# PKU-EPIC/GraspNeRF

Hardware: AMD Instinct MI355X
Metric: scenes/sec TSDF+render fwd, 6-view 40^3 grid (higher is better)
Workload: dtype f32

## Files before the change

### graspnerf_amd/_lib.py

```python
import ctypes as C
import os

_HERE = os.path.dirname(os.path.abspath(__file__))
LIB_PATH = os.path.join(_HERE, 'csrc', os.environ.get('GNR_LIB', 'libgnr.so'))

GNR_OK, GNR_ERR_ARG, GNR_ERR_SHAPE, GNR_ERR_HIP, GNR_ERR_WORKSPACE = 0, -1, -2, -3, -4
ERRORS = {-1: 'GNR_ERR_ARG', -2: 'GNR_ERR_SHAPE', -3: 'GNR_ERR_HIP', -4: 'GNR_ERR_WORKSPACE'}

c_float_p = C.POINTER(C.c_float)


class GnrScene(C.Structure):
    _fields_ = [('B', C.c_int), ('V', C.c_int), ('H', C.c_int), ('W', C.c_int), ('fh', C.c_int), ('fw', C.c_int),
                ('imgs', C.c_void_p), ('img_feats', C.c_void_p), ('ray_feats', C.c_void_p),
                ('poses', C.c_void_p), ('Ks', C.c_void_p), ('depth_range', C.c_void_p), ('use_vis', C.c_int), ('options', C.c_uint)]


OPTIONS = {'fp32_chain': 0x001, 'feature_grad_fixed': 0x002, 'view1_one_wavefront': 0x004, 'view2_one_wavefront': 0x008,
           'ray_order_morton': 0x010, 'poison_partials': 0x020, 'direct_scatter': 0x040, 'geo_dual_fp32': 0x080, 'test_lose_partner': 0x100, 'static_tiles': 0x200, 'split_launch': 0x400,
           'sample_order_natural': 0x800}
GNR_STATUS_LOST_PARTNER = 16


class GnrRays(C.Structure):
# ... 51 lines not shown
        getattr(L, name).argtypes = [C.c_void_p, C.c_void_p, C.c_void_p]
        getattr(L, name).restype = C.c_int
    L.gnr_layout_offset.argtypes = [C.c_char_p]
    L.gnr_layout_offset.restype = C.c_int
    L.gnr_workspace_bytes.argtypes = [C.POINTER(GnrScene), C.c_int, C.c_int, C.c_int]
    L.gnr_workspace_bytes.restype = C.c_size_t
    L.gnr_prepare.argtypes = [C.POINTER(GnrScene), C.c_void_p, C.c_size_t, C.c_void_p]
    L.gnr_prepare.restype = C.c_int
    L.gnr_range_status.argtypes = [C.POINTER(GnrScene), C.c_void_p, C.c_size_t, C.POINTER(C.c_uint), C.c_void_p]
    L.gnr_range_status.restype = C.c_int
    L.gnr_status_words_offset.argtypes = [C.POINTER(GnrScene)]
    L.gnr_status_words_offset.restype = C.c_size_t
    L.gnr_sample_volume_fwd.argtypes = [C.POINTER(GnrScene), C.c_void_p, C.c_int, C.c_void_p, C.c_void_p,
                                        C.c_void_p, C.c_void_p, C.c_size_t, C.c_void_p]
    L.gnr_sample_volume_fwd.restype = C.c_int
    L.gnr_debug_volume_chain.argtypes = [C.POINTER(GnrScene), C.c_void_p, C.c_int, C.c_void_p, C.c_void_p,
                                         C.c_void_p, C.c_size_t, C.c_void_p]
    L.gnr_debug_volume_chain.restype = C.c_int
    L.gnr_depth_mean_fwd.argtypes = [C.POINTER(GnrScene), C.c_void_p, C.c_int, C.c_void_p, C.c_void_p,
                                     C.c_void_p, C.c_size_t, C.c_void_p]
    L.gnr_depth_mean_fwd.restype = C.c_int
    L.gnr_merge_depths.argtypes = [C.c_void_p, C.c_int, C.c_void_p, C.c_int, C.c_void_p, C.c_int, C.c_void_p]
    L.gnr_merge_depths.restype = C.c_int
    L.gnr_render_by_depth_fwd.argtypes = [C.POINTER(GnrScene), C.POINTER(GnrRays), C.c_void_p, C.c_int, C.c_void_p,
                                          C.POINTER(GnrRenderOut), C.c_void_p, C.c_size_t, C.c_void_p]
    L.gnr_render_by_depth_fwd.restype = C.c_int
    L.gnr_debug_render_by_depth_perm.argtypes = [C.POINTER(GnrScene), C.POINTER(GnrRays), C.c_void_p, C.c_int, C.c_void_p,
                                                 C.POINTER(GnrRenderOut), C.c_void_p, C.c_void_p, C.c_size_t, C.c_void_p]
    L.gnr_debug_render_by_depth_perm.restype = C.c_int
    L.gnr_debug_sample_order.argtypes = [C.c_void_p, C.c_int, C.c_int, C.c_void_p, C.c_void_p]
    L.gnr_debug_sample_order.restype = C.c_int
    L.gnr_sample_order_host.argtypes = [C.c_void_p, C.c_int, C.c_void_p]
    L.gnr_sample_order_host.restype = C.c_int
    L.gnr_sample_order_offsets.argtypes = [C.POINTER(GnrScene), C.c_int, C.c_int, C.POINTER(C.c_size_t), C.POINTER(C.c_size_t)]
    L.gnr_sample_order_offsets.restype = C.c_int
    L.gnr_render_rays_fwd.argtypes = [C.POINTER(GnrScene), C.POINTER(GnrRays), C.c_void_p, C.c_void_p,
                                      C.POINTER(GnrRenderOut), C.POINTER(GnrRenderOut), C.c_void_p, C.c_void_p,
                                      C.c_void_p, C.c_size_t, C.c_void_p]
    L.gnr_render_rays_fwd.restype = C.c_int
    L.gnr_head_canonical_floats.restype = C.c_int
    L.gnr_head_packed_floats.restype = C.c_int
    L.gnr_pack_grasp_head.argtypes = [c_float_p, c_float_p]
    L.gnr_pack_grasp_head.restype = C.c_int
    L.gnr_grasp_head_workspace_bytes.argtypes = [C.c_int, C.c_int]
    L.gnr_grasp_head_workspace_bytes.restype = C.c_size_t
    L.gnr_grasp_head_fwd.argtypes = [C.c_int, C.c_int, C.c_void_p, C.c_void_p, C.c_void_p, C.c_void_p, C.c_void_p,
                                     C.c_void_p, C.c_size_t, C.c_void_p]
    L.gnr_grasp_head_fwd.restype = C.c_int
    L.gnr_head_last_error.restype = C.c_char_p
    L.gnr_conv3d_bwd_weight.argtypes = [C.c_void_p] * 3 + [C.c_int] * 7 + [C.c_void_p]
    L.gnr_conv3d_same_bwd_weight.argtypes = [C.c_void_p] * 3 + [C.c_int] * 7 + [C.c_void_p, C.c_size_t, C.c_void_p]
    L.gnr_conv3d_same_bwd_weight_workspace_bytes.argtypes = [C.c_int] * 7
    L.gnr_conv3d_same_bwd_weight_workspace_bytes.restype = C.c_size_t
    L.gnr_conv3d_same_bwd_weight.restype = C.c_int
    L.gnr_conv3d_same_workspace_bytes.argtypes = [C.c_int] * 3
    L.gnr_conv3d_same_workspace_bytes.restype = C.c_size_t
    L.gnr_conv3d_same.argtypes = [C.c_void_p] * 4 + [C.c_int] * 8 + [C.c_void_p, C.c_size_t, C.c_void_p]
    L.gnr_conv3d_same.restype = C.c_int
    L.gnr_conv3d_tap_mask_words.argtypes = [C.c_int] * 2
    L.gnr_conv3d_tap_mask_words.restype = C.c_size_t
    L.gnr_conv3d_tap_mask.argtypes = [C.c_void_p, C.c_void_p, C.c_int, C.c_int, C.c_int, C.c_void_p]
    L.gnr_conv3d_tap_mask.restype = C.c_int
    L.gnr_conv3d_same_masked.argtypes = [C.c_void_p] * 4 + [C.c_int] * 8 + [C.c_void_p, C.c_void_p, C.c_size_t, C.c_void_p]
    L.gnr_conv3d_same_masked.restype = C.c_int
    L.gnr_conv3d_same_bwd_weight_masked.argtypes = [C.c_void_p] * 3 + [C.c_int] * 7 + [C.c_void_p, C.c_void_p, C.c_size_t, C.c_void_p]
    L.gnr_conv3d_same_bwd_weight_masked.restype = C.c_int
# ... 61 lines not shown
    L.gnr_timing_begin_only.argtypes = [C.c_char_p]
    L.gnr_timing_begin_only.restype = C.c_int
    L.gnr_timing_end.argtypes = [C.c_char_p, C.c_size_t]
    L.gnr_timing_end.restype = C.c_int
    L.gnr_chain_timing_end.argtypes = [c_float_p, C.POINTER(C.c_int)]
    L.gnr_chain_timing_end.restype = C.c_int
    L.gnr_img_last_error.restype = C.c_char_p
    L.gnr_instnorm_act.argtypes = [C.c_void_p] * 7 + [C.c_longlong, C.c_int, C.c_int, C.c_float, C.c_int, C.c_void_p]
    L.gnr_instnorm_act.restype = C.c_int
    L.gnr_instnorm_act_bwd.argtypes = [C.c_void_p] * 12 + [C.c_longlong, C.c_int, C.c_int, C.c_int, C.c_void_p]
    L.gnr_instnorm_act_bwd.restype = C.c_int
    for fn in (L.gnr_reflect_pad2d, L.gnr_reflect_pad2d_bwd):
        fn.argtypes = [C.c_void_p, C.c_void_p, C.c_longlong, C.c_int, C.c_int, C.c_int, C.c_void_p]
        fn.restype = C.c_int
    L.gnr_upsample2x_bilinear.argtypes = [C.c_void_p, C.c_void_p, C.c_longlong, C.c_int, C.c_int, C.c_void_p]
    L.gnr_upsample2x_bilinear.restype = C.c_int
    L.gnr_ingest_tables_bytes.argtypes = [C.c_int, C.c_int]
    L.gnr_ingest_tables_bytes.restype = C.c_size_t
    L.gnr_ingest_tables_host.argtypes = [C.c_int] * 4 + [C.c_void_p]
    L.gnr_ingest_tables_host.restype = C.c_int
    L.gnr_ingest_u8.argtypes = [C.c_void_p] + [C.c_int] * 4 + [C.c_size_t, C.c_size_t, C.c_void_p, C.c_void_p, C.c_int, C.c_int, C.c_void_p]
    L.gnr_ingest_u8.restype = C.c_int
    L.gnr_ingest_last_error.restype = C.c_char_p
    L.gnr_last_error.restype = C.c_char_p
    L.gnr_dominant_kernel_name.restype = C.c_char_p
    L.gnr_debug_fill_lds.argtypes = [C.c_uint, C.c_void_p]
    L.gnr_debug_fill_lds.restype = C.c_int
    _lib = L
    return L


EXPORTED = ['gnr_canonical_weights_floats', 'gnr_packed_weights_floats', 'gnr_pack_weights', 'gnr_pack_vis_decoder', 'gnr_pack_vis_decoder_bwd', 'gnr_canonical_vis_floats', 'gnr_pack_weights_device', 'gnr_pack_weights_bwd_device', 'gnr_pack_vis_decoder_device', 'gnr_pack_vis_decoder_bwd_device', 'gnr_layout_offset', 'gnr_workspace_bytes',
            'gnr_prepare', 'gnr_range_status', 'gnr_status_words_offset', 'gnr_sample_volume_fwd', 'gnr_debug_volume_chain', 'gnr_depth_mean_fwd', 'gnr_merge_depths', 'gnr_render_by_depth_fwd', 'gnr_render_rays_fwd',
            'gnr_debug_render_by_depth_perm', 'gnr_debug_sample_order', 'gnr_sample_order_host', 'gnr_sample_order_offsets',
            'gnr_dominant_kernel_name', 'gnr_last_error', 'gnr_time_chain_kernel', 'gnr_head_canonical_floats',
            'gnr_head_packed_floats', 'gnr_pack_grasp_head', 'gnr_grasp_head_workspace_bytes', 'gnr_grasp_head_fwd',
            'gnr_head_last_error', 'gnr_chain_timing_begin', 'gnr_chain_timing_end', 'gnr_timing_begin', 'gnr_timing_begin_only', 'gnr_timing_end', 'gnr_grasp_select_workspace_bytes',
            'gnr_grasp_select_fwd', 'gnr_post_last_error', 'gnr_packed_bwd_floats', 'gnr_pack_weights_bwd',
            'gnr_depth_mean_bwd_workspace_bytes', 'gnr_depth_mean_bwd', 'gnr_sample_volume_train_workspace_bytes',
            'gnr_train_workspace_layout', 'gnr_sample_volume_fwd_train', 'gnr_sample_volume_bwd',
            'gnr_render_chain_train_workspace_bytes', 'gnr_render_chain_fwd_train', 'gnr_render_chain_bwd', 'gnr_conv3d_bwd_weight', 'gnr_conv3d_same_workspace_bytes', 'gnr_conv3d_same', 'gnr_conv3d_tap_mask_words', 'gnr_conv3d_tap_mask', 'gnr_conv3d_same_masked', 'gnr_conv3d_same_bwd_weight_masked', 'gnr_conv3d_same_bwd_weight', 'gnr_conv3d_same_bwd_weight_workspace_bytes',
            'gnr_render_tail_fwd_train', 'gnr_ray_tail_grad_floats', 'gnr_ray_tail_dual_bwd', 'gnr_ray_tail_dual_bwd_workspace_bytes', 'gnr_composite_bwd', 'gnr_composite_bwd_workspace_bytes', 'gnr_geo_dual_fwd', 'gnr_geo_dual_fwd_workspace_bytes', 'gnr_geo_dual_bwd', 'gnr_geo_dual_bwd_workspace_bytes', 'gnr_host_randperm_prefix',
            'gnr_debug_fill_lds', 'gnr_img_last_error', 'gnr_instnorm_act', 'gnr_instnorm_act_bwd', 'gnr_reflect_pad2d', 'gnr_reflect_pad2d_bwd', 'gnr_upsample2x_bilinear',
            'gnr_ingest_tables_bytes', 'gnr_ingest_tables_host', 'gnr_ingest_u8', 'gnr_ingest_last_error']


def check(rc, what):
    if rc != GNR_OK:
        msg = lib().gnr_last_error().decode(errors='replace')
        raise GnrError(f'{what} failed: {ERRORS.get(rc, rc)} ({msg})')


def timing_begin(only=None):
    check(lib().gnr_timing_begin_only(only.encode() if only else None), 'gnr_timing_begin')


def timing_end():
    buf = C.create_string_buffer(1 << 16)
    n = lib().gnr_timing_end(buf, len(buf))
    if n < 0:
        check(n, 'gnr_timing_end')
    out = {}
    for line in buf.value.decode().splitlines():
        label, cnt, ms = line.rsplit(' ', 2)
        out[label] = (int(cnt), float(ms))
    return out
```

### graspnerf_amd/csrc/gnr_capi.inc

```
#include <stdio.h>
#include <string.h>
#include <atomic>
#include <mutex>
#include <type_traits>

#include "../../include/gnr.h"

namespace gnr {

static thread_local char g_err[512] = "";
static int fail(int code, const char* what, hipError_t e = hipSuccess) {
    snprintf(g_err, sizeof(g_err), "%s%s%s", what, e != hipSuccess ? ": " : "", e != hipSuccess ? hipGetErrorString(e) : "");
    return code;
}
#define GNR_HIP(call)                                                         \
    do {                                                                      \
        hipError_t e_ = (call);                                               \
        if (e_ != hipSuccess) return fail(GNR_ERR_HIP, #call, e_);            \
    } while (0)

static inline size_t al256(size_t x) { return (x + 255) & ~(size_t)255; }

static bool attr_needed(std::atomic<unsigned long long>& done) {
    int dev = 0;
// ... 453 lines not shown
}

extern "C" int gnr_sample_volume_fwd(const GnrScene* s, const float* bbox_min, int R, const float* wc, float* sdf_out,
                                     unsigned char* vmask_out, void* ws, size_t ws_bytes, void* stream) {
    if (int rc = check_scene(s)) return rc;
    if (!bbox_min || !wc || !sdf_out || !ws) return fail(GNR_ERR_ARG, "gnr_sample_volume_fwd: null pointer");
    if (R < 2 || R > MAX_DN) return fail(GNR_ERR_SHAPE, "volume_res must be in 2..64");
    return volume_impl(s, bbox_min, R, wc, sdf_out, vmask_out, ws, ws_bytes, (hipStream_t)stream, true, true, true);
}

extern "C" int gnr_debug_volume_chain(const GnrScene* s, const float* bbox_min, int R, const float* wc, float* dbg,
                                      void* ws, size_t ws_bytes, void* stream) {
    if (int rc = check_scene(s)) return rc;
    if (!bbox_min || !wc || !dbg || !ws) return fail(GNR_ERR_ARG, "gnr_debug_volume_chain: null pointer");
    return volume_impl(s, bbox_min, R, wc, nullptr, nullptr, ws, ws_bytes, (hipStream_t)stream, true, true, false, dbg);
}

static int order_rays(const GnrScene* s, const GnrRays* q, Workspace& w, hipStream_t st, const int** perm_out) {
    *perm_out = nullptr;
    if (!opt(s, GNR_OPT_RAY_ORDER_MORTON) || q->rn > MAX_SORT_RAYS || q->rn < 2) return GNR_OK;
    int shift = 0;
    while (((s->W > s->H ? s->W : s->H) >> shift) > 1024) ++shift;
    if (int rc = launch<k_ray_order>("k_ray_order@render_pass", st, dim3(s->B), dim3(256), 0, q->coords, w.ray_perm, q->rn, shift)) return rc;
    *perm_out = w.ray_perm;
    return GNR_OK;
}

constexpr int SAMPLE_ORDER_MIN_TILES_PER_SLOT = 8;
static bool sample_order_wanted(const GnrScene* s, const Workspace& w, int P) {
    if (opt(s, GNR_OPT_SAMPLE_ORDER_NATURAL) || !w.sample_perm || !w.sample_keys || P > MAX_SORT_SAMPLES) return false;
    const long ntiles = (long)s->B * ((P + 15) / 16), slots = (long)num_cus() * (GNR_CHAIN_THREADS / 64);
    return ntiles >= SAMPLE_ORDER_MIN_TILES_PER_SLOT * slots;
}
static int launch_sample_order(const unsigned char* keys, int* perm, int B, int P, int nkeys, hipStream_t st) {
    return launch<k_sample_order>("k_sample_order@render_pass", st, dim3(B), dim3(1024), 0, keys, perm, P, nkeys);
}
static RayArgs render_ray_args(const GnrScene* s, const GnrRays* q, const float* depth, int dn, const float* wl, const GnrRenderOut* out,
                               const Workspace& w, const float* desc) {
    RayArgs r;
    memset(&r, 0, sizeof(r));
    r.wpk = wl; r.rec = w.rec; r.desc = desc; r.depth = depth; r.colors = out->colors_nr; r.que_dr = q->que_depth_range;
    r.nrays = s->B * q->rn; r.dn = dn; r.rays_per_scene = q->rn;
    r.sdf = out->sdf_values; r.alpha = out->alpha_values; r.hit = out->hit_prob_nr; r.pix = out->pixel_colors_nr;
    r.rdepth = out->render_depth; r.gerr_part = out->sdf_gradient_error ? w.gerr_part : nullptr; r.grad = out->sdf_gradient;
    r.rmask = out->ray_mask; r.view_num = q->ray_mask_view_num; r.point_num = q->ray_mask_point_num;
    r.range_word = w.range_flag ? w.range_flag + RS_RAY_WATCH : nullptr;
    return r;
}
static int render_ray_epilogue(const GnrScene* s, const GnrRays* q, const GnrRenderOut* out, int dn, const Workspace& w, const char* gerr_label,
                               const char* gt_label, bool want_gt, float* gt_also, hipStream_t st) {
    const int B = s->B, rn = q->rn;
    if (out->sdf_gradient_error) {
        const int chunk = q->ray_batch_num > 0 ? q->ray_batch_num : rn;
        if (int rc = launch<k_gerr_reduce>(gerr_label, st, dim3(B, (rn + chunk - 1) / chunk), dim3(256), 0, w.gerr_part, out->sdf_gradient_error, rn, dn, chunk)) return rc;
    }
    if (out->pixel_colors_gt && q->que_imgs && want_gt)
        if (int rc = launch<k_pixel_gt>(gt_label, st, dim3((B * rn + 255) / 256), dim3(256), 0, q->que_imgs, q->coords, out->pixel_colors_gt, rn, s->H, s->W, B, gt_also)) return rc;
    return GNR_OK;
}
static int render_pass(const GnrScene* s, const GnrRays* q, const float* depth, int dn, const float* wl, GnrRenderOut* out,
                       Workspace& w, hipStream_t st, float* fine_depth, int* fine_inds, int fdn, const float* fine_u = nullptr,
                       const int* perm = nullptr, int range_slot = RS_COARSE, float* gt_also = nullptr, bool skip_gt = false, bool gen_depth = false,
                       const int* sample_perm_in = nullptr) {
    if (!out || !out->colors_nr) return fail(GNR_ERR_ARG, "GnrRenderOut.colors_nr is required");
    const int B = s->B, rn = q->rn;
    const int P = rn * dn;
    const bool ordered = !sample_perm_in && sample_order_wanted(s, w, P);
    if (int rc = launch<k_points_rays>("k_points_rays@render_pass", st, dim3((B * P + 255) / 256), dim3(256), 0, q->coords, q->que_pose, q->que_K,
                                       q->que_depth_range, depth, w.desc, rn, dn, B, perm, gen_depth ? const_cast<float*>(depth) : nullptr,
                                       ordered ? w.sample_keys : nullptr, w.viewp, s->V, s->H, s->W)) return rc;
    if (ordered)
        if (int rc = launch_sample_order(w.sample_keys, w.sample_perm, B, P, 1 << s->V, st)) return rc;
    ChainArgs a{wl, w.feat64, s->imgs, w.viewp, w.desc, w.rec, out->colors_nr, out->view_mask, nullptr,
                B, P, s->H, s->W, s->fh, s->fw, 0};
    wire_chain(a, s, w, range_slot);
    a.ray_perm = perm; a.perm_rn = rn; a.perm_dn = dn;
    a.sample_perm = ordered ? w.sample_perm : sample_perm_in;
    if (int rc = launch_chain<true>(s, a, st)) return rc;
    RayArgs r = render_ray_args(s, q, depth, dn, wl, out, w, w.desc);
    r.fine_depth = fine_depth; r.fine_inds = fine_inds; r.fdn = fdn; r.fine_u = fine_u; r.ray_perm = perm;
    if (int rc = launch_ray<true>(r, st)) return rc;
    if (int rc = render_ray_epilogue(s, q, out, dn, w, "k_gerr_reduce@render_pass", "k_pixel_gt@render_pass", !skip_gt, gt_also, st)) return rc;
    if (out->depth && out->depth != depth)
        GNR_HIP(hipMemcpyAsync(out->depth, depth, (size_t)B * P * sizeof(float), hipMemcpyDeviceToDevice, st));
    return GNR_OK;
}

static int check_rays(const GnrRays* q, bool by_depth = false) {
    if (!q || !q->coords || !q->que_pose || !q->que_K || !q->que_depth_range) return fail(GNR_ERR_ARG, "GnrRays: null pointer");
    if (q->rn < 1) return fail(GNR_ERR_SHAPE, "GnrRays: rn must be positive");
    if (!by_depth && (q->dn < 3 || q->dn > MAX_DN || q->fdn < 1 || q->fdn > MAX_DN)) return fail(GNR_ERR_SHAPE, "GnrRays: dn/fdn must be in 3..64");
    if (q->fine_depth_use_all != 0 && q->fine_depth_use_all != 1) return fail(GNR_ERR_ARG, "GnrRays: fine_depth_use_all must be 0 or 1");
    if (q->ray_batch_num < 0) return fail(GNR_ERR_SHAPE, "GnrRays: ray_batch_num must be >= 0");
    return GNR_OK;
}

extern "C" int gnr_render_by_depth_fwd(const GnrScene* s, const GnrRays* q, const float* depth, int dn, const float* wl,
                                       GnrRenderOut* out, void* ws, size_t ws_bytes, void* stream) {
    if (int rc = check_scene(s)) return rc;
    if (int rc = check_rays(q, true)) return rc;
    if (!depth || !wl || !ws) return fail(GNR_ERR_ARG, "gnr_render_by_depth_fwd: null pointer");
    if (dn < 3 || dn > MAX_DN_FWD) return fail(GNR_ERR_SHAPE, "dn must be in 3..128");
    if (int rc = check_points(s, (size_t)q->rn * dn)) return rc;
    Workspace w = carve(s, (size_t)q->rn * dn, q->rn, ws);
    if (ws_bytes < w.total) return fail(GNR_ERR_WORKSPACE, "workspace too small");
    const int* perm = nullptr;
    if (int rc = order_rays(s, q, w, (hipStream_t)stream, &perm)) return rc;
    return render_pass(s, q, depth, dn, wl, out, w, (hipStream_t)stream, nullptr, nullptr, 0, nullptr, perm);
}

extern "C" int gnr_debug_render_by_depth_perm(const GnrScene* s, const GnrRays* q, const float* depth, int dn, const float* wl,
                                              GnrRenderOut* out, const int* sample_perm, void* ws, size_t ws_bytes, void* stream) {
    if (int rc = check_scene(s)) return rc;
    if (int rc = check_rays(q, true)) return rc;
    if (!depth || !wl || !ws || !sample_perm) return fail(GNR_ERR_ARG, "gnr_debug_render_by_depth_perm: null pointer");
    if (dn < 3 || dn > MAX_DN_FWD) return fail(GNR_ERR_SHAPE, "dn must be in 3..128");
    if (int rc = check_points(s, (size_t)q->rn * dn)) return rc;
    Workspace w = carve(s, (size_t)q->rn * dn, q->rn, ws);
    if (ws_bytes < w.total) return fail(GNR_ERR_WORKSPACE, "workspace too small");
    const int* perm = nullptr;
    if (int rc = order_rays(s, q, w, (hipStream_t)stream, &perm)) return rc;
    return render_pass(s, q, depth, dn, wl, out, w, (hipStream_t)stream, nullptr, nullptr, 0, nullptr, perm, RS_COARSE, nullptr, false, false, sample_perm);
}

extern "C" int gnr_debug_sample_order(const unsigned char* keys, int B, int P, int* perm, void* stream) {
    if (!keys || !perm) return fail(GNR_ERR_ARG, "gnr_debug_sample_order: null pointer");
    if (B < 1 || P < 1 || P > MAX_SORT_SAMPLES) return fail(GNR_ERR_SHAPE, "gnr_debug_sample_order: 1 <= P <= 2^18 samples per scene");
    return launch_sample_order(keys, perm, B, P, 256, (hipStream_t)stream);
}
extern "C" int gnr_sample_order_host(const unsigned char* keys, int P, int* perm_out) {
    if (!keys || !perm_out) return fail(GNR_ERR_ARG, "gnr_sample_order_host: null pointer");
    if (P < 1) return fail(GNR_ERR_SHAPE, "gnr_sample_order_host: P must be positive");
    int start[256], hist[256] = {0};
    for (int i = 0; i < P; ++i) ++hist[keys[i]];
    for (int k = 0; k < 256; ++k) {
        start[k] = 0;
        for (int k2 = 0; k2 < 256; ++k2) if (sorder::key_before(k2, k)) start[k] += hist[k2];
    }
    for (int i = 0; i < P; ++i) perm_out[sorder::slot_of(start[keys[i]]++, P)] = i;
    return GNR_OK;
}
extern "C" int gnr_sample_order_offsets(const GnrScene* s, int rn, int dn_max, size_t* keys_off, size_t* perm_off) {
    if (!s || !keys_off || !perm_off) return fail(GNR_ERR_ARG, "gnr_sample_order_offsets: null pointer");
    if (rn < 1 || dn_max < 1) return fail(GNR_ERR_SHAPE, "gnr_sample_order_offsets: rn, dn_max must be positive");
    char* const base = (char*)4096;
    Workspace w = carve(s, (size_t)rn * dn_max, rn, base);
    if ((size_t)rn * dn_max > (size_t)MAX_SORT_SAMPLES) return fail(GNR_ERR_SHAPE, "gnr_sample_order_offsets: more samples per scene than the sort handles");
    *keys_off = (size_t)((char*)w.sample_keys - base); *perm_off = (size_t)((char*)w.sample_perm - base);
    return GNR_OK;
}

extern "C" int gnr_render_rays_fwd(const GnrScene* s, const GnrRays* q, const float* wc, const float* wf, GnrRenderOut* coarse,
                                   GnrRenderOut* fine, const float* fine_depth_in, int* fine_inds_out, void* ws, size_t ws_bytes,
                                   void* stream) {
    if (int rc = check_scene(s)) return rc;
    if (int rc = check_rays(q)) return rc;
    if (!wc || !coarse || !ws || (fine && !wf)) return fail(GNR_ERR_ARG, "gnr_render_rays_fwd: null pointer");
    if (!fine && (fine_depth_in || fine_inds_out)) return fail(GNR_ERR_ARG, "gnr_render_rays_fwd: fine depths / indices without a fine pass");
    hipStream_t st = (hipStream_t)stream;
    const int fine_dn = !fine ? 0 : (q->fine_depth_use_all ? q->dn + q->fdn : q->fdn);
    const int dmax = q->dn > fine_dn ? q->dn : fine_dn;
    if (int rc = check_points(s, (size_t)q->rn * dmax)) return rc;
    Workspace w = carve(s, (size_t)q->rn * dmax, q->rn, ws);
    if (ws_bytes < w.total) return fail(GNR_ERR_WORKSPACE, "workspace too small");
    const int B = s->B;
    float* depth_c = coarse->depth ? coarse->depth : w.depth_c;
    const int* perm = nullptr;
    if (int rc = order_rays(s, q, w, st, &perm)) return rc;
    if (!fine) return render_pass(s, q, depth_c, q->dn, wc, coarse, w, st, nullptr, nullptr, 0, nullptr, perm, RS_COARSE, nullptr, false, true);
    float* depth_f = (fine->depth && !fine_depth_in && !q->fine_depth_use_all) ? fine->depth : w.depth_f;
    const bool one_gt = coarse->pixel_colors_gt && fine->pixel_colors_gt && q->que_imgs && coarse->pixel_colors_gt != fine->pixel_colors_gt;
    if (int rc = render_pass(s, q, depth_c, q->dn, wc, coarse, w, st, depth_f, fine_inds_out, q->fdn, q->fine_u, perm, RS_COARSE,
// ... 583 lines not shown
```

### graspnerf_amd/csrc/gnr_kernels.hip

```cpp
#include <hip/hip_runtime.h>
#include <stdint.h>
#include <type_traits>

#include "gnr_layout.h"
#include "gnr_sample_order.h"

#ifndef GNR_ABLATE
#define GNR_ABLATE 0
#endif

namespace gnr {

typedef float f4 __attribute__((ext_vector_type(4)));
typedef float f2 __attribute__((ext_vector_type(2)));

#define DEV __device__ __forceinline__

DEV f4 mfma16(float a, float b, f4 c) { return __builtin_amdgcn_mfma_f32_16x16x4f32(a, b, c, 0, 0, 0); }
DEV float elu1(float x) { return fmaxf(x, __builtin_amdgcn_fmed3f(__expf(x), 0.f, 1.f) - 1.f); }
constexpr float kLog2e = 1.4426950408889634f, kLn2 = 0.6931471805599453f;
#if GNR_ABLATE & 8
DEV float elu_s(float xs) { return xs; }
#else
DEV float elu_s(float xs) { return fmaxf(xs, fmaf(__builtin_amdgcn_fmed3f(__builtin_amdgcn_exp2f(xs), 0.f, 1.f), kLog2e, -kLog2e)); }
// ... 555 lines not shown
    };
    assemble(0, 1, o.f);
    assemble(2, 3, o.i);
}
DEV void view_dir(const float* __restrict__ vp, const float (&p)[3], const float (&qd)[3], float (&dd)[4]) {
    float d[3] = {p[0] - vp[12], p[1] - vp[13], p[2] - vp[14]};
    const float inr = -__builtin_amdgcn_rsqf(fmaxf(d[0] * d[0] + d[1] * d[1] + d[2] * d[2], 1e-10f));
    d[0] *= inr; d[1] *= inr; d[2] *= inr;
    dd[0] = d[0] - qd[0]; dd[1] = d[1] - qd[1]; dd[2] = d[2] - qd[2];
    dd[3] = d[0] * qd[0] + d[1] * qd[1] + d[2] * qd[2];
}

constexpr int SW = 20;
#ifndef GNR_TWO_QUEUES
#define GNR_TWO_QUEUES 0
#endif
#ifndef GNR_RDF2_PAIRS
#define GNR_RDF2_PAIRS 0
#endif
constexpr int rows_a(int V) { return GNR_TWO_QUEUES ? (V + 1) / 2 : V; }
constexpr int rows_b(int V) { return GNR_TWO_QUEUES ? V / 2 : 0; }

DEV unsigned view_mask_key(const float* __restrict__ viewp_b, const float (&p)[3], int V, int H, int W) {
    const float qd[3] = {0.f, 0.f, 0.f};
    unsigned k = 0;
    for (int v = 0; v < V; ++v) {
        ViewGeom vg;
        project_view<false>(viewp_b + v * VIEWP_FLOATS, p, qd, H, W, vg);
        k |= (vg.m != 0.f ? 1u : 0u) << v;
    }
    return k;
}
constexpr int MAX_SORT_SAMPLES = 1 << 18;
constexpr int SO_DEPTH = 16;
__global__ __launch_bounds__(1024) void k_sample_order(const unsigned char* __restrict__ keys, int* __restrict__ perm, int P, int nkeys) {
    __shared__ int hist[256];
    __shared__ int wbase[16][256];
    const int tid = threadIdx.x, lane = tid & 63, wave = tid >> 6;
    const unsigned char* kb = keys + (size_t)blockIdx.x * P;
    int* pb = perm + (size_t)blockIdx.x * P;
    for (int i = tid; i < 16 * 256; i += 1024) (&wbase[0][0])[i] = 0;
    __syncthreads();
    const int seg = ((P + 16 * 64 - 1) / (16 * 64)) * 64;
    const int s0 = min(P, wave * seg), s1 = min(P, s0 + seg);
    for (int i0 = s0; i0 < s1; i0 += 64 * SO_DEPTH) {
        int kk[SO_DEPTH];
#pragma unroll
        for (int u = 0; u < SO_DEPTH; ++u) { const int i = i0 + u * 64 + lane; kk[u] = i < s1 ? (int)kb[i] : -1; }
#pragma unroll
        for (int u = 0; u < SO_DEPTH; ++u) if (kk[u] >= 0) atomicAdd(&wbase[wave][kk[u]], 1);
    }
    __syncthreads();
    if (tid < nkeys) {
        int t = 0;
        for (int w = 0; w < 16; ++w) t += wbase[w][tid];
        hist[tid] = t;
    }
    __syncthreads();
    if (tid < nkeys) {
        int run = 0;
        for (int k2 = 0; k2 < nkeys; ++k2) if (sorder::key_before(k2, tid)) run += hist[k2];
        for (int w = 0; w < 16; ++w) { const int c = wbase[w][tid]; wbase[w][tid] = run; run += c; }
    }
    __syncthreads();
    volatile int* base = wbase[wave];
    for (int i0 = s0; i0 < s1; i0 += 64 * SO_DEPTH) {
        int kk[SO_DEPTH];
#pragma unroll
        for (int u = 0; u < SO_DEPTH; ++u) { const int i = i0 + u * 64 + lane; kk[u] = i < s1 ? (int)kb[i] : -1; }
#pragma unroll
        for (int u = 0; u < SO_DEPTH; ++u) {
            if (i0 + u * 64 >= s1) break;
            const int k = kk[u];
            const bool ok = k >= 0;
            unsigned long long same = __ballot(ok);
#pragma unroll
            for (int bit = 0; bit < 8; ++bit) {
                const bool on = (k >> bit) & 1;
                const unsigned long long bb = __ballot(on);
                same &= on ? bb : ~bb;
            }
            const int rank = __popcll(same & ((1ull << lane) - 1ull));
            const int pos = ok ? base[k] + rank : 0;
            __builtin_amdgcn_wave_barrier();
            if (ok && rank == 0) base[k] = pos + __popcll(same);
            __builtin_amdgcn_wave_barrier();
            if (ok) pb[sorder::slot_of(pos, P)] = i0 + u * 64 + lane;
        }
    }
}

#ifndef GNR_DYN_TILES
#define GNR_DYN_TILES 1
#endif
#ifndef GNR_VOLUME_POINTS_INLINE
#define GNR_VOLUME_POINTS_INLINE 1
#endif
#ifndef GNR_TAIL_OLD_ONLY
#define GNR_TAIL_OLD_ONLY 0
#endif
#ifndef GNR_DESC_PREFETCH
#define GNR_DESC_PREFETCH 0
#endif
#ifndef GNR_DYN_CTR_INC
#define GNR_DYN_CTR_INC 0
#endif
#ifndef GNR_DYN_TRAIN
#define GNR_DYN_TRAIN 1
#endif
#ifndef GNR_SKIP_MASKED
#define GNR_SKIP_MASKED 1
#endif
#ifndef GNR_CHAIN_THREADS
#define GNR_CHAIN_THREADS 512
#endif
#define GNR_CHAIN_MIN_BLOCKS (GNR_CHAIN_THREADS >= 1024 ? 1 : GNR_CHAIN_THREADS / 256)
#ifndef GNR_WAVE_CLOCK
#define GNR_WAVE_CLOCK 0
#endif
#if GNR_WAVE_CLOCK
__device__ unsigned long long g_wave_clock[2][4096][8];
__device__ unsigned g_tile_clock[2][1 << 17];
// ... 1388 lines not shown
```

### graspnerf_amd/csrc/gnr_sample_order.h

```cpp
#pragma once

#if defined(__HIPCC__)
#define GNR_SO_HD __host__ __device__
#else
#define GNR_SO_HD
#endif

namespace gnr {
namespace sorder {

constexpr int STRIPES = 8;
constexpr int TILE = 16;

GNR_SO_HD inline int popcount8(int k) { k = (k & 0x55) + ((k >> 1) & 0x55); k = (k & 0x33) + ((k >> 2) & 0x33); return (k & 0x0f) + (k >> 4); }

GNR_SO_HD inline bool key_before(int a, int b) {
    const int pa = popcount8(a), pb = popcount8(b);
    return pa != pb ? pa > pb : a > b;
}

GNR_SO_HD inline int stripe_tiles(int tps, int s) { return (tps - s + STRIPES - 1) / STRIPES; }

GNR_SO_HD inline int slot_of(int pos, int P) {
    const int tps = (P + TILE - 1) / TILE;
    const int rem = P - (tps - 1) * TILE;
    const int gshort = tps <= STRIPES ? tps - 1 : STRIPES * (tps / STRIPES) - 1;
    int gi, wi;
    if (pos < TILE * gshort) { gi = pos / TILE; wi = pos % TILE; }
    else if (pos < TILE * gshort + rem) { gi = gshort; wi = pos - TILE * gshort; }
    else { const int q = pos + TILE - rem; gi = q / TILE; wi = q % TILE; }
    const int s = gi % STRIPES;
    int tile = gi / STRIPES;
    for (int k = 0; k < s; ++k) tile += stripe_tiles(tps, k);
    return tile * TILE + wi;
}

}
}
```

### include/gnr.h

```cpp
#ifndef GNR_H
#define GNR_H
#include <stddef.h>

#ifdef __cplusplus
extern "C" {
#endif

#define GNR_OK 0
#define GNR_ERR_ARG (-1)
#define GNR_ERR_SHAPE (-2)
#define GNR_ERR_HIP (-3)
#define GNR_ERR_WORKSPACE (-4)

typedef struct GnrScene {
    int B, V;
    int H, W;
    int fh, fw;
    const float* imgs;
    const float* img_feats;
    const float* ray_feats;
    const float* poses;
    const float* Ks;
    const float* depth_range;
    int use_vis;
// ... 53 lines not shown
int gnr_canonical_vis_floats(void);
int gnr_pack_weights_device(const float* canonical_dev, float* packed_dev, void* stream);
int gnr_pack_weights_bwd_device(const float* canonical_dev, float* packed_bwd_dev, void* stream);
int gnr_pack_vis_decoder_device(const float* vis_decoder_dev, float* packed_dev, void* stream);
int gnr_pack_vis_decoder_bwd_device(const float* vis_decoder_dev, float* packed_bwd_dev, void* stream);
int gnr_layout_offset(const char* name);

size_t gnr_workspace_bytes(const GnrScene* scene, int volume_res, int rn, int dn_max);

int gnr_prepare(const GnrScene* scene, void* workspace, size_t workspace_bytes, void* stream);

#define GNR_STATUS_LOST_PARTNER 16u
int gnr_range_status(const GnrScene* scene, const void* workspace, size_t workspace_bytes, unsigned* flags_out, void* stream);
size_t gnr_status_words_offset(const GnrScene* scene);

int gnr_sample_volume_fwd(const GnrScene* scene, const float* bbox_min , int volume_res,
                          const float* packed_coarse , float* sdf_out ,
                          unsigned char* view_mask_out, void* workspace, size_t workspace_bytes,
                          void* stream);

int gnr_render_by_depth_fwd(const GnrScene* scene, const GnrRays* rays, const float* depth, int dn,
                            const float* level_weights, GnrRenderOut* out, void* workspace,
                            size_t workspace_bytes, void* stream);

int gnr_render_rays_fwd(const GnrScene* scene, const GnrRays* rays, const float* packed_coarse,
                        const float* packed_fine, GnrRenderOut* coarse, GnrRenderOut* fine,
                        const float* fine_depth_in, int* fine_inds_out, void* workspace,
                        size_t workspace_bytes, void* stream);

int gnr_debug_render_by_depth_perm(const GnrScene* scene, const GnrRays* rays, const float* depth, int dn, const float* level_weights,
                                   GnrRenderOut* out, const int* sample_perm, void* workspace, size_t workspace_bytes, void* stream);
int gnr_debug_sample_order(const unsigned char* keys, int B, int P, int* perm, void* stream);
int gnr_sample_order_host(const unsigned char* keys_host, int P, int* perm_out_host);
int gnr_sample_order_offsets(const GnrScene* scene, int rn, int dn_max, size_t* keys_offset, size_t* perm_offset);

int gnr_merge_depths(const float* depth_a, int na, const float* depth_b, int nb, float* out, int nrays, void* stream);

int gnr_depth_mean_fwd(const GnrScene* scene, const float* coords, int pn, const float* level_weights,
                       float* mean_out, void* workspace, size_t workspace_bytes, void* stream);

int gnr_debug_volume_chain(const GnrScene* scene, const float* bbox_min, int volume_res,
                           const float* packed_coarse, float* dbg, void* workspace,
                           size_t workspace_bytes, void* stream);

int gnr_head_canonical_floats(void);
int gnr_head_packed_floats(void);
int gnr_pack_grasp_head(const float* canonical_host, float* packed_host);
size_t gnr_grasp_head_workspace_bytes(int B, int volume_res);
int gnr_grasp_head_fwd(int B, int volume_res, const float* volume, const float* packed_head, float* qual, float* rot,
                       float* width, void* workspace, size_t workspace_bytes, void* stream);
const char* gnr_head_last_error(void);
int gnr_conv3d_bwd_weight(const float* x, const float* dy, float* dw, int B, int Cin, int Cout, int D, int H, int W, int K,
                          void* stream);

size_t gnr_conv3d_same_workspace_bytes(int Cin, int Cout, int K);
size_t gnr_conv3d_same_bwd_weight_workspace_bytes(int B, int Cin, int Cout, int D, int H, int W, int K);
int gnr_conv3d_same_bwd_weight(const float* x, const float* dy, float* dw, int B, int Cin, int Cout, int D, int H, int W, int K,
                               void* workspace, size_t workspace_bytes, void* stream);
int gnr_conv3d_same(const float* x, const float* w, const float* bias, float* y, int B, int Cin, int Cout, int D, int H, int W, int K,
                    int mode, void* workspace, size_t workspace_bytes, void* stream);
#define GNR_CONV3D_FIRST_GEN 0x100
size_t gnr_conv3d_tap_mask_words(int Cin, int Cout);
int gnr_conv3d_tap_mask(const float* pattern, unsigned* mask, int Cin, int Cout, int K, void* stream);
int gnr_conv3d_same_masked(const float* x, const float* w, const float* bias, float* y, int B, int Cin, int Cout, int D, int H, int W,
                           int K, int mode, const unsigned* mask, void* workspace, size_t workspace_bytes, void* stream);
int gnr_conv3d_same_bwd_weight_masked(const float* x, const float* dy, float* dw, int B, int Cin, int Cout, int D, int H, int W, int K,
// ... 105 lines not shown
```

Baseline: 5132.

## Parallelize sample-order counting sort across chunked blocks per scene

The sample ordering kernel previously ran one 1024-thread block per scene, counting and scattering all samples serially per wave. It now launches a grid of chunks per scene. Each block redundantly histograms the whole key array using vectorized 16-byte loads with run-length counting, splits counts into before and in-chunk, then ranks and scatters only its own chunk. A parallel LDS prefix scan replaces the per-key serial loop. This trades redundant global histogram reads for much more parallelism, and it adds a host reference for the chunked ordering.

```diff
diff --git a/graspnerf_amd/_lib.py b/graspnerf_amd/_lib.py
--- a/graspnerf_amd/_lib.py
+++ b/graspnerf_amd/_lib.py
@@ -107,6 +107,8 @@
     L.gnr_debug_sample_order.restype = C.c_int
     L.gnr_sample_order_host.argtypes = [C.c_void_p, C.c_int, C.c_void_p]
     L.gnr_sample_order_host.restype = C.c_int
+    L.gnr_sample_order_host_chunked.argtypes = [C.c_void_p, C.c_int, C.c_int, C.c_void_p]
+    L.gnr_sample_order_host_chunked.restype = C.c_int
     L.gnr_sample_order_offsets.argtypes = [C.POINTER(GnrScene), C.c_int, C.c_int, C.POINTER(C.c_size_t), C.POINTER(C.c_size_t)]
     L.gnr_sample_order_offsets.restype = C.c_int
     L.gnr_render_rays_fwd.argtypes = [C.POINTER(GnrScene), C.POINTER(GnrRays), C.c_void_p, C.c_void_p,
@@ -234,7 +236,7 @@
 
 EXPORTED = ['gnr_canonical_weights_floats', 'gnr_packed_weights_floats', 'gnr_pack_weights', 'gnr_pack_vis_decoder', 'gnr_pack_vis_decoder_bwd', 'gnr_canonical_vis_floats', 'gnr_pack_weights_device', 'gnr_pack_weights_bwd_device', 'gnr_pack_vis_decoder_device', 'gnr_pack_vis_decoder_bwd_device', 'gnr_layout_offset', 'gnr_workspace_bytes',
             'gnr_prepare', 'gnr_range_status', 'gnr_status_words_offset', 'gnr_sample_volume_fwd', 'gnr_debug_volume_chain', 'gnr_depth_mean_fwd', 'gnr_merge_depths', 'gnr_render_by_depth_fwd', 'gnr_render_rays_fwd',
-            'gnr_debug_render_by_depth_perm', 'gnr_debug_sample_order', 'gnr_sample_order_host', 'gnr_sample_order_offsets',
+            'gnr_debug_render_by_depth_perm', 'gnr_debug_sample_order', 'gnr_sample_order_host', 'gnr_sample_order_host_chunked', 'gnr_sample_order_offsets',
             'gnr_dominant_kernel_name', 'gnr_last_error', 'gnr_time_chain_kernel', 'gnr_head_canonical_floats',
             'gnr_head_packed_floats', 'gnr_pack_grasp_head', 'gnr_grasp_head_workspace_bytes', 'gnr_grasp_head_fwd',
             'gnr_head_last_error', 'gnr_chain_timing_begin', 'gnr_chain_timing_end', 'gnr_timing_begin', 'gnr_timing_begin_only', 'gnr_timing_end', 'gnr_grasp_select_workspace_bytes',
diff --git a/graspnerf_amd/csrc/gnr_capi.inc b/graspnerf_amd/csrc/gnr_capi.inc
--- a/graspnerf_amd/csrc/gnr_capi.inc
+++ b/graspnerf_amd/csrc/gnr_capi.inc
@@ -509,8 +509,8 @@
     const long ntiles = (long)s->B * ((P + 15) / 16), slots = (long)num_cus() * (GNR_CHAIN_THREADS / 64);
     return ntiles >= SAMPLE_ORDER_MIN_TILES_PER_SLOT * slots;
 }
-static int launch_sample_order(const unsigned char* keys, int* perm, int B, int P, int nkeys, hipStream_t st) {
-    return launch<k_sample_order>("k_sample_order@render_pass", st, dim3(B), dim3(1024), 0, keys, perm, P, nkeys);
+static int launch_sample_order(const unsigned char* keys, int* perm, int B, int P, hipStream_t st) {
+    return launch<k_sample_order>("k_sample_order@render_pass", st, dim3((P + SO_CHUNK - 1) / SO_CHUNK, B), dim3(SO_THREADS), 0, keys, perm, P);
 }
 static RayArgs render_ray_args(const GnrScene* s, const GnrRays* q, const float* depth, int dn, const float* wl, const GnrRenderOut* out,
                                const Workspace& w, const float* desc) {
@@ -547,7 +547,7 @@
                                        q->que_depth_range, depth, w.desc, rn, dn, B, perm, gen_depth ? const_cast<float*>(depth) : nullptr,
                                        ordered ? w.sample_keys : nullptr, w.viewp, s->V, s->H, s->W)) return rc;
     if (ordered)
-        if (int rc = launch_sample_order(w.sample_keys, w.sample_perm, B, P, 1 << s->V, st)) return rc;
+        if (int rc = launch_sample_order(w.sample_keys, w.sample_perm, B, P, st)) return rc;
     ChainArgs a{wl, w.feat64, s->imgs, w.viewp, w.desc, w.rec, out->colors_nr, out->view_mask, nullptr,
                 B, P, s->H, s->W, s->fh, s->fw, 0};
     wire_chain(a, s, w, range_slot);
@@ -603,7 +603,7 @@
 extern "C" int gnr_debug_sample_order(const unsigned char* keys, int B, int P, int* perm, void* stream) {
     if (!keys || !perm) return fail(GNR_ERR_ARG, "gnr_debug_sample_order: null pointer");
     if (B < 1 || P < 1 || P > MAX_SORT_SAMPLES) return fail(GNR_ERR_SHAPE, "gnr_debug_sample_order: 1 <= P <= 2^18 samples per scene");
-    return launch_sample_order(keys, perm, B, P, 256, (hipStream_t)stream);
+    return launch_sample_order(keys, perm, B, P, (hipStream_t)stream);
 }
 extern "C" int gnr_sample_order_host(const unsigned char* keys, int P, int* perm_out) {
     if (!keys || !perm_out) return fail(GNR_ERR_ARG, "gnr_sample_order_host: null pointer");
@@ -615,6 +615,18 @@
         for (int k2 = 0; k2 < 256; ++k2) if (sorder::key_before(k2, k)) start[k] += hist[k2];
     }
     for (int i = 0; i < P; ++i) perm_out[sorder::slot_of(start[keys[i]]++, P)] = i;
+    return GNR_OK;
+}
+extern "C" int gnr_sample_order_host_chunked(const unsigned char* keys, int P, int chunk, int* perm_out) {
+    if (!keys || !perm_out) return fail(GNR_ERR_ARG, "gnr_sample_order_host_chunked: null pointer");
+    if (P < 1 || chunk < 1) return fail(GNR_ERR_SHAPE, "gnr_sample_order_host_chunked: P and chunk must be positive");
+    for (int c0 = 0; c0 < P; c0 += chunk) {
+        int before[sorder::KEYS] = {0}, rest[sorder::KEYS] = {0}, by_rank[sorder::KEYS], scan[sorder::KEYS], in_chunk[sorder::KEYS] = {0};
+        for (int i = 0; i < P; ++i) ++(i < c0 ? before : rest)[keys[i]];
+        for (int k = 0; k < sorder::KEYS; ++k) by_rank[sorder::key_rank(k)] = before[k] + rest[k];
+        for (int r = 0, run = 0; r < sorder::KEYS; ++r) { scan[r] = run; run += by_rank[r]; }
+        for (int i = c0; i < P && i - c0 < chunk; ++i) perm_out[sorder::slot_of(sorder::chunk_pos(scan, before, keys[i], in_chunk[keys[i]]++), P)] = i;
+    }
     return GNR_OK;
 }
 extern "C" int gnr_sample_order_offsets(const GnrScene* s, int rn, int dn_max, size_t* keys_off, size_t* perm_off) {
diff --git a/graspnerf_amd/csrc/gnr_kernels.hip b/graspnerf_amd/csrc/gnr_kernels.hip
--- a/graspnerf_amd/csrc/gnr_kernels.hip
+++ b/graspnerf_amd/csrc/gnr_kernels.hip
@@ -611,62 +611,104 @@
     return k;
 }
 constexpr int MAX_SORT_SAMPLES = 1 << 18;
-constexpr int SO_DEPTH = 16;
-__global__ __launch_bounds__(1024) void k_sample_order(const unsigned char* __restrict__ keys, int* __restrict__ perm, int P, int nkeys) {
-    __shared__ int hist[256];
-    __shared__ int wbase[16][256];
+constexpr int SO_THREADS = 1024;
+constexpr int SO_STEPS = 4;
+constexpr int SO_CHUNK = SO_THREADS * SO_STEPS;
+constexpr int SO_LOADS = 4;
+DEV void so_count_word(const uint4& q, int i0, int c0, int P, int* cnt) {
+    const unsigned d[4] = {q.x, q.y, q.z, q.w};
+    unsigned starts = 0x10001u;
+#pragma unroll
+    for (int n = 0; n < 4; ++n) {
+        const unsigned t = d[n] ^ ((d[n] << 8) | (n ? d[n - 1] >> 24 : 0u));
+        const unsigned m = ((((t & 0x7f7f7f7fu) + 0x7f7f7f7fu) | t) & 0x80808080u) >> 7;
+        starts |= (((m * 0x00204081u) >> 21) & 15u) << (4 * n);
+    }
+    const int edge[3] = {-i0, c0 - i0, P - i0};
+#pragma unroll
+    for (int e = 0; e < 3; ++e) starts |= (unsigned)edge[e] < 16u ? 1u << edge[e] : 0u;
+    for (int j = 0; j < 16;) {
+        starts &= starts - 1u;
+        const int jn = __builtin_ctz(starts), i = i0 + j;
+        const unsigned w = j < 8 ? (j < 4 ? d[0] : d[1]) : (j < 12 ? d[2] : d[3]);
+        if ((unsigned)i < (unsigned)P) atomicAdd(&cnt[(int)((w >> (8 * (j & 3))) & 255u) + (i >= c0 ? sorder::KEYS : 0)], jn - j);
+        j = jn;
+    }
+}
+__global__ __launch_bounds__(SO_THREADS) void k_sample_order(const unsigned char* __restrict__ keys, int* __restrict__ perm, int P) {
+    constexpr int WAVES = SO_THREADS / 64, SCAN_WAVES = sorder::KEYS / 64;
+    static_assert(SO_THREADS % 64 == 0 && SO_THREADS >= sorder::KEYS && SO_THREADS <= 1024, "one thread per key");
+    __shared__ int cnt[2 * sorder::KEYS];
+    __shared__ int wbase[WAVES][sorder::KEYS];
+    __shared__ int scan[sorder::KEYS];
+    __shared__ int wtot[SCAN_WAVES];
     const int tid = threadIdx.x, lane = tid & 63, wave = tid >> 6;
-    const unsigned char* kb = keys + (size_t)blockIdx.x * P;
-    int* pb = perm + (size_t)blockIdx.x * P;
-    for (int i = tid; i < 16 * 256; i += 1024) (&wbase[0][0])[i] = 0;
+    const unsigned char* kb = keys + (size_t)blockIdx.y * P;
+    int* pb = perm + (size_t)blockIdx.y * P;
+    const int c0 = blockIdx.x * SO_CHUNK;
+    const int s0 = c0 + wave * (64 * SO_STEPS) + lane;
+    int kk[SO_STEPS];
+#pragma unroll
+    for (int u = 0; u < SO_STEPS; ++u) kk[u] = s0 + 64 * u < P ? (int)kb[s0 + 64 * u] : -1;
+    const int shift = (int)((size_t)kb & 15);
+    const uint4* wp = (const uint4*)(kb - shift);
+    const int nwords = (shift + P + 15) >> 4;
+    uint4 q[SO_LOADS];
+#pragma unroll
+    for (int u = 0; u < SO_LOADS; ++u) { const int w = tid + u * SO_THREADS; q[u] = w < nwords ? wp[w] : make_uint4(0, 0, 0, 0); }
+    for (int n = tid; n < 2 * sorder::KEYS; n += SO_THREADS) cnt[n] = 0;
+    for (int n = tid; n < WAVES * sorder::KEYS; n += SO_THREADS) (&wbase[0][0])[n] = 0;
     __syncthreads();
-    const int seg = ((P + 16 * 64 - 1) / (16 * 64)) * 64;
-    const int s0 = min(P, wave * seg), s1 = min(P, s0 + seg);
-    for (int i0 = s0; i0 < s1; i0 += 64 * SO_DEPTH) {
-        int kk[SO_DEPTH];
-#pragma unroll
-        for (int u = 0; u < SO_DEPTH; ++u) { const int i = i0 + u * 64 + lane; kk[u] = i < s1 ? (int)kb[i] : -1; }
-#pragma unroll
-        for (int u = 0; u < SO_DEPTH; ++u) if (kk[u] >= 0) atomicAdd(&wbase[wave][kk[u]], 1);
+    for (int w0 = tid; w0 < nwords; w0 += SO_LOADS * SO_THREADS) {
+        if (w0 != tid) {
+#pragma unroll
+            for (int u = 0; u < SO_LOADS; ++u) { const int w = w0 + u * SO_THREADS; q[u] = w < nwords ? wp[w] : make_uint4(0, 0, 0, 0); }
+        }
+#pragma unroll
+        for (int u = 0; u < SO_LOADS; ++u) { const int w = w0 + u * SO_THREADS; if (w < nwords) so_count_word(q[u], w * 16 - shift, c0, P, cnt); }
+    }
+    int rank[SO_STEPS];
+#pragma unroll
+    for (int u = 0; u < SO_STEPS; ++u) {
+        const int k = kk[u];
+        const bool ok = k >= 0;
+        unsigned long long same = __ballot(ok);
+#pragma unroll
+        for (int bit = 0; bit < 8; ++bit) {
+            const bool on = (k >> bit) & 1;
+            const unsigned long long bb = __ballot(on);
+            same &= on ? bb : ~bb;
+        }
+        const int r = __popcll(same & ((1ull << lane) - 1ull));
+        int seen = 0;
+        if (ok && r == 0) seen = atomicAdd(&wbase[wave][k], __popcll(same));
+        rank[u] = r + __shfl(seen, ok ? __builtin_ctzll(same) : lane);
     }
     __syncthreads();
-    if (tid < nkeys) {
-        int t = 0;
-        for (int w = 0; w < 16; ++w) t += wbase[w][tid];
-        hist[tid] = t;
-    }
+    if (tid < sorder::KEYS) scan[sorder::key_rank(tid)] = cnt[tid] + cnt[sorder::KEYS + tid];
     __syncthreads();
-    if (tid < nkeys) {
-        int run = 0;
-        for (int k2 = 0; k2 < nkeys; ++k2) if (sorder::key_before(k2, tid)) run += hist[k2];
-        for (int w = 0; w < 16; ++w) { const int c = wbase[w][tid]; wbase[w][tid] = run; run += c; }
+    int h = 0, incl = 0;
+    if (tid < sorder::KEYS) {
+        h = incl = scan[tid];
+#pragma unroll
+        for (int d = 1; d < 64; d <<= 1) { const int t = __shfl_up(incl, d); if (lane >= d) incl += t; }
+        if (lane == 63) wtot[wave] = incl;
     }
     __syncthreads();
-    volatile int* base = wbase[wave];
-    for (int i0 = s0; i0 < s1; i0 += 64 * SO_DEPTH) {
-        int kk[SO_DEPTH];
-#pragma unroll
-        for (int u = 0; u < SO_DEPTH; ++u) { const int i = i0 + u * 64 + lane; kk[u] = i < s1 ? (int)kb[i] : -1; }
-#pragma unroll
-        for (int u = 0; u < SO_DEPTH; ++u) {
-            if (i0 + u * 64 >= s1) break;
-            const int k = kk[u];
-            const bool ok = k >= 0;
-            unsigned long long same = __ballot(ok);
-#pragma unroll
-            for (int bit = 0; bit < 8; ++bit) {
-                const bool on = (k >> bit) & 1;
-                const unsigned long long bb = __ballot(on);
-                same &= on ? bb : ~bb;
-            }
-            const int rank = __popcll(same & ((1ull << lane) - 1ull));
-            const int pos = ok ? base[k] + rank : 0;
-            __builtin_amdgcn_wave_barrier();
-            if (ok && rank == 0) base[k] = pos + __popcll(same);
-            __builtin_amdgcn_wave_barrier();
-            if (ok) pb[sorder::slot_of(pos, P)] = i0 + u * 64 + lane;
-        }
-    }
+    if (tid < sorder::KEYS) {
+        int off = 0;
+        for (int w = 0; w < wave; ++w) off += wtot[w];
+        scan[tid] = off + incl - h;
+    }
+    __syncthreads();
+    if (tid < sorder::KEYS) {
+        int run = sorder::chunk_pos(scan, cnt, tid, 0);
+        for (int w = 0; w < WAVES; ++w) { const int c = wbase[w][tid]; wbase[w][tid] = run; run += c; }
+    }
+    __syncthreads();
+#pragma unroll
+    for (int u = 0; u < SO_STEPS; ++u)
+        if (kk[u] >= 0) pb[sorder::slot_of(wbase[wave][kk[u]] + rank[u], P)] = s0 + 64 * u;
 }
 
 #ifndef GNR_DYN_TILES
diff --git a/graspnerf_amd/csrc/gnr_sample_order.h b/graspnerf_amd/csrc/gnr_sample_order.h
--- a/graspnerf_amd/csrc/gnr_sample_order.h
+++ b/graspnerf_amd/csrc/gnr_sample_order.h
@@ -12,12 +12,29 @@
 constexpr int STRIPES = 8;
 constexpr int TILE = 16;
 
-GNR_SO_HD inline int popcount8(int k) { k = (k & 0x55) + ((k >> 1) & 0x55); k = (k & 0x33) + ((k >> 2) & 0x33); return (k & 0x0f) + (k >> 4); }
+GNR_SO_HD constexpr int popcount8(int k) { k = (k & 0x55) + ((k >> 1) & 0x55); k = (k & 0x33) + ((k >> 2) & 0x33); return (k & 0x0f) + (k >> 4); }
 
-GNR_SO_HD inline bool key_before(int a, int b) {
+GNR_SO_HD constexpr bool key_before(int a, int b) {
     const int pa = popcount8(a), pb = popcount8(b);
     return pa != pb ? pa > pb : a > b;
 }
+
+constexpr int KEYS = 256;
+struct KeyRanks { unsigned char r[KEYS]; };
+constexpr KeyRanks make_key_ranks() {
+    KeyRanks t{};
+    for (int k = 0; k < KEYS; ++k) {
+        int n = 0;
+        for (int k2 = 0; k2 < KEYS; ++k2) n += key_before(k2, k) ? 1 : 0;
+        t.r[k] = (unsigned char)n;
+    }
+    return t;
+}
+GNR_SO_HD inline int key_rank(int k) {
+    constexpr KeyRanks t = make_key_ranks();
+    return t.r[k];
+}
+GNR_SO_HD inline int chunk_pos(const int* scan, const int* before, int k, int rank_in_chunk) { return scan[key_rank(k)] + before[k] + rank_in_chunk; }
 
 GNR_SO_HD inline int stripe_tiles(int tps, int s) { return (tps - s + STRIPES - 1) / STRIPES; }
 
diff --git a/include/gnr.h b/include/gnr.h
--- a/include/gnr.h
+++ b/include/gnr.h
@@ -109,6 +109,7 @@
                                    GnrRenderOut* out, const int* sample_perm, void* workspace, size_t workspace_bytes, void* stream);
 int gnr_debug_sample_order(const unsigned char* keys, int B, int P, int* perm, void* stream);
 int gnr_sample_order_host(const unsigned char* keys_host, int P, int* perm_out_host);
+int gnr_sample_order_host_chunked(const unsigned char* keys_host, int P, int chunk, int* perm_out_host);
 int gnr_sample_order_offsets(const GnrScene* scene, int rn, int dn_max, size_t* keys_offset, size_t* perm_offset);
 
 int gnr_merge_depths(const float* depth_a, int na, const float* depth_b, int nb, float* out, int nrays, void* stream);
```

New measurement: 5191 (median of 6 runs). +1.2%, better.
